# 959AI994/Multi-Gate-VAE

Hardware: NVIDIA B200
Metric: gates_per_s_fwd_bwd (higher is better)
Workload: dtype f32

## Files before the change

multi-gate-vae_b200/csrc/linear.cu:

```cuda
#include "mgv_common.cuh"

namespace {

constexpr int RG = 8;

template <int TO, int TI, int LR>
__global__ void __launch_bounds__(256) linear_wgrad_kernel(const float* __restrict__ x, const float* __restrict__ gy, long long N,
                                                           int I, int O, int IP, int OP, float* __restrict__ partial) {
    extern __shared__ __align__(16) float sm[];
    const int stage_floats = LR * (IP + OP);
    const int tid = threadIdx.x, nt = blockDim.x;
    const int ntx = IP / TI, tx = tid % ntx, ty = tid / ntx;
    const bool active = ty < OP / TO;
    float acc[TO][TI];
    float bsum[TO];
#pragma unroll
    for (int a = 0; a < TO; ++a) {
        bsum[a] = 0.f;
#pragma unroll
        for (int b = 0; b < TI; ++b) acc[a][b] = 0.f;
    }
    const long long trips = (N + LR - 1) / LR;
    const long long t0 = trips * blockIdx.x / gridDim.x, t1 = trips * (blockIdx.x + 1) / gridDim.x;
    const bool vec = (I == IP) && (O == OP) && (I % 4 == 0) && (O % 4 == 0);
    auto stage = [&](long long t, int buf) {
        float* Xs = sm + buf * stage_floats;
        float* Gs = Xs + LR * IP;
        const long long r0 = t * LR;
        const int rows = (int)((N - r0 < LR) ? (N - r0) : LR);
        if (vec) {
            const float* xs = x + r0 * I;
            const float* gs = gy + r0 * O;
            for (int q = tid; q < LR * I / 4; q += nt) {
                const unsigned src = (q < rows * I / 4) ? 16u : 0u;
                asm volatile("cp.async.cg.shared.global [%0], [%1], 16, %2;" ::"r"((unsigned)__cvta_generic_to_shared(Xs + 4 * q)),
                             "l"(src ? xs + 4 * q : x), "r"(src) : "memory");
            }
            for (int q = tid; q < LR * O / 4; q += nt) {
                const unsigned src = (q < rows * O / 4) ? 16u : 0u;
                asm volatile("cp.async.cg.shared.global [%0], [%1], 16, %2;" ::"r"((unsigned)__cvta_generic_to_shared(Gs + 4 * q)),
                             "l"(src ? gs + 4 * q : gy), "r"(src) : "memory");
            }
        } else {
            for (int q = tid; q < LR * IP; q += nt) {
                const int r = q / IP, c = q % IP;
                Xs[q] = (r < rows && c < I) ? x[(r0 + r) * I + c] : 0.f;
            }
            for (int q = tid; q < LR * OP; q += nt) {
                const int r = q / OP, c = q % OP;
                Gs[q] = (r < rows && c < O) ? gy[(r0 + r) * O + c] : 0.f;
            }
        }
        asm volatile("cp.async.commit_group;" ::: "memory");
    };
    if (t0 < t1) stage(t0, 0);
    for (long long t = t0; t < t1; ++t) {
        const int buf = (int)((t - t0) & 1);
        if (t + 1 < t1) {
            stage(t + 1, buf ^ 1);
            asm volatile("cp.async.wait_group 1;" ::: "memory");
        } else {
            asm volatile("cp.async.wait_group 0;" ::: "memory");
        }
        __syncthreads();
        const float* Xs = sm + buf * stage_floats;
        const float* Gs = Xs + LR * IP;
        if (active) {
#pragma unroll 4
            for (int r = 0; r < LR; ++r) {
                float g[TO], xv[TI];
#pragma unroll
                for (int a = 0; a < TO; a += 4) *reinterpret_cast<float4*>(&g[a]) = *reinterpret_cast<const float4*>(Gs + r * OP + TO * ty + a);
#pragma unroll
                for (int b = 0; b < TI; b += 4) *reinterpret_cast<float4*>(&xv[b]) = *reinterpret_cast<const float4*>(Xs + r * IP + (b / 4) * (IP / 2) + 4 * tx);
#pragma unroll
                for (int a = 0; a < TO; ++a) {
                    bsum[a] += g[a];
#pragma unroll
                    for (int b = 0; b < TI; ++b) acc[a][b] = fmaf(g[a], xv[b], acc[a][b]);
                }
            }
        }
        __syncthreads();
    }
    if (!active) return;
    float* P = partial + (size_t)blockIdx.x * ((size_t)O * I + O);
#pragma unroll
    for (int a = 0; a < TO; ++a) {
        const int o = TO * ty + a;
        if (o < O) {
#pragma unroll
            for (int b = 0; b < TI; ++b) {
                const int i = (b / 4) * (IP / 2) + 4 * tx + (b & 3);
                if (i < I) P[(size_t)o * I + i] = acc[a][b];
            }
            if (tx == 0) P[(size_t)O * I + o] = bsum[a];
        }
    }
}

__global__ void __launch_bounds__(256) linear_wgrad_reduce_kernel(const float* __restrict__ partial, int nblk, int I, int O,
                                                                  float* __restrict__ dW, float* __restrict__ db) {
    __shared__ float red[RG][32];
    const int total = O * I + O;
    const int j = threadIdx.x & 31, g = threadIdx.x >> 5;
    const int i = blockIdx.x * 32 + j;
    float s = 0.f;
    if (i < total) {
#pragma unroll 4
        for (int b = g; b < nblk; b += RG) s += partial[(size_t)b * total + i];
    }
    red[g][j] = s;
    __syncthreads();
    if (g == 0 && i < total) {
#pragma unroll
        for (int k = 1; k < RG; ++k) s += red[k][j];
        if (i < O * I) dW[i] = s;
        else if (db) db[i - O * I] = s;
    }
}

int grid_blocks(long long N) {
    int dev = 0, sms = 148;
    cudaGetDevice(&dev);
    cudaDeviceGetAttribute(&sms, cudaDevAttrMultiProcessorCount, dev);
    long long trips = (N + 127) / 128;
    long long g = 2LL * sms;
    if (g > trips) g = trips;
    return g < 1 ? 1 : (int)g;
}

template <int TO, int TI, int LR>
int launch(int nblk, cudaStream_t st, const float* x, const float* gy, long long N, int I, int O, float* partial) {
    const int IP = (I + TI - 1) / TI * TI, OP = (O + TO - 1) / TO * TO;
    int nt = (IP / TI) * (OP / TO);
    nt = nt < 256 ? 256 : (nt + 31) / 32 * 32;
    const size_t smem = 2 * (size_t)LR * (IP + OP) * sizeof(float);
    MGV_CUDA(cudaFuncSetAttribute((const void*)linear_wgrad_kernel<TO, TI, LR>, cudaFuncAttributeMaxDynamicSharedMemorySize, (int)smem));
    linear_wgrad_kernel<TO, TI, LR><<<nblk, nt, smem, st>>>(x, gy, N, I, O, IP, OP, partial);
    return MGV_OK;
}

}

extern "C" size_t mgv_linear_wgrad_workspace_bytes(int64_t N, int32_t I, int32_t O) {
    return (size_t)grid_blocks(N) * ((size_t)O * I + O) * sizeof(float) + 256;
}

extern "C" int mgv_linear_wgrad(const float* x, const float* gy, int64_t N, int32_t I, int32_t O, float* dW, float* db,
                                void* ws, size_t ws_bytes, mgv_stream_t stream) {
    cudaStream_t st = (cudaStream_t)stream;
    MGV_REQUIRE(I >= 1 && I <= 128 && O >= 1 && O <= 128, "mgv_linear_wgrad: in/out features must be in 1..128 (got %d, %d)", I, O);
    MGV_REQUIRE(N >= 0 && dW != nullptr, "mgv_linear_wgrad: bad argument");
    if (N == 0) {
        MGV_CUDA(cudaMemsetAsync(dW, 0, (size_t)O * I * sizeof(float), st));
        if (db) MGV_CUDA(cudaMemsetAsync(db, 0, (size_t)O * sizeof(float), st));
        return MGV_OK;
    }
    if (ws_bytes < mgv_linear_wgrad_workspace_bytes(N, I, O)) {
        mgv_set_error("mgv_linear_wgrad: workspace %zu < %zu bytes", ws_bytes, mgv_linear_wgrad_workspace_bytes(N, I, O));
        return MGV_ERR_WORKSPACE;
    }
    const int nblk = grid_blocks(N);
    float* partial = (float*)ws;
    const bool o8 = O > 32, i8 = I > 32;
    int rc;
    if (o8 && i8) rc = launch<8, 8, 64>(nblk, st, x, gy, N, I, O, partial);
    else if (o8) rc = launch<8, 4, 128>(nblk, st, x, gy, N, I, O, partial);
    else if (i8) rc = launch<4, 8, 128>(nblk, st, x, gy, N, I, O, partial);
    else rc = launch<4, 4, 128>(nblk, st, x, gy, N, I, O, partial);
    if (rc != MGV_OK) return rc;
    const int total = O * I + O;
    linear_wgrad_reduce_kernel<<<(total + 31) / 32, 256, 0, st>>>(partial, nblk, I, O, dW, db);
    mgv_count_launches(2);
    return mgv_check_cuda(cudaGetLastError(), "mgv_linear_wgrad");
}
```

multi-gate-vae_b200/csrc/readout.cu:

```cuda
#include "mgv_common.cuh"

namespace {

constexpr int DI = MGV_D, DH = 32;
constexpr int RD_THREADS = 256, RD_WARPS = RD_THREADS / 32;
constexpr int NB = 4;

struct RdParams {
    const float *W1, *b1, *g1, *be1, *W2, *b2, *g2, *be2, *W3, *b3;
    float *rm1, *rv1, *rm2, *rv2;
};
struct RdFwd {
    RdParams P;
    const float* x; long long N;
    int training; float p_drop; unsigned long long seed; float momentum, eps;
    const float* target;
    float* pred; float* loss;
    float* saved;
    float* stats;
    unsigned* mask;
    double* acc;
    unsigned* bar;
};
struct RdBwd {
    RdParams P;
    const float* x; long long N;
    int training; float p_drop; unsigned long long seed;
    const float* target; const float* saved; const float* stats;
    const float* g_pred;
    const float* g_loss;
    float* gx;
    float* grads;
    float* dz1;
    float* partial;
    double* acc;
    unsigned* bar;
};
constexpr int G_W1 = 0, G_B1 = 2048, G_G1 = 2080, G_BE1 = 2112, G_W2 = 2144, G_B2 = 3168, G_G2 = 3200, G_BE2 = 3232, G_W3 = 3264, G_B3 = 3296;

__device__ __forceinline__ float keep_scale(unsigned long long seed, long long n, int layer, int c, float p, float sc) {
    if (p <= 0.f) return 1.0f;
    uint32_t h = (uint32_t)(n * 64 + layer * 32 + c) ^ (uint32_t)seed;
    h ^= h >> 16; h *= 0x85EBCA6Bu; h ^= h >> 13; h *= 0xC2B2AE35u; h ^= h >> 16;
    h += (uint32_t)(seed >> 32) + (uint32_t)(n >> 26);
    h ^= h >> 15; h *= 0x2C1B3C6Du; h ^= h >> 12; h *= 0x297A2D39u; h ^= h >> 15;
    const float u = (float)(h >> 8) * (1.0f / 16777216.0f);
    return u >= p ? sc : 0.f;
}
__device__ __forceinline__ float warp_sum(float v) {
#pragma unroll
    for (int o = 16; o > 0; o >>= 1) v += __shfl_xor_sync(0xffffffffu, v, o);
    return v;
}
__device__ __forceinline__ float dot64(const float* xs, const float (&w)[DI], float b) {
    float a0 = b, a1 = 0.f;
#pragma unroll
    for (int k = 0; k < DI; k += 4) {
        const float4 v = *reinterpret_cast<const float4*>(xs + k);
        a0 = fmaf(v.x, w[k], a0); a1 = fmaf(v.y, w[k + 1], a1);
        a0 = fmaf(v.z, w[k + 2], a0); a1 = fmaf(v.w, w[k + 3], a1);
    }
    return a0 + a1;
}
__device__ __forceinline__ float dot32(float h, const float (&w)[DH], float b) {
    float a0 = b, a1 = 0.f;
#pragma unroll
    for (int j = 0; j < DH; j += 2) {
        a0 = fmaf(__shfl_sync(0xffffffffu, h, j), w[j], a0);
        a1 = fmaf(__shfl_sync(0xffffffffu, h, j + 1), w[j + 1], a1);
    }
    return a0 + a1;
}

__global__ void __launch_bounds__(RD_THREADS, 2) readout_fwd_kernel(const RdFwd p) {
    __shared__ __align__(16) float xs[RD_WARPS][NB][DI];
    __shared__ double red[RD_WARPS][2][DH];
    const int lane = threadIdx.x & 31, warp = threadIdx.x >> 5;
    const long long gw = (long long)blockIdx.x * RD_WARPS + warp, nw = (long long)gridDim.x * RD_WARPS;
    const RdParams& P = p.P;
    const float sc = p.p_drop > 0.f ? 1.0f / (1.0f - p.p_drop) : 1.0f;
    const bool train = p.training != 0;
    float w[DI];
#pragma unroll
    for (int k = 0; k < DI; ++k) w[k] = __ldg(P.W1 + lane * DI + k);
    const float b1 = __ldg(P.b1 + lane);
    double s = 0.0, q = 0.0;
    for (long long n0 = gw * NB; n0 < p.N; n0 += nw * NB) {
#pragma unroll
        for (int i = 0; i < NB; ++i)
            if (n0 + i < p.N) *reinterpret_cast<float2*>(&xs[warp][i][2 * lane]) = __ldg(reinterpret_cast<const float2*>(p.x + (n0 + i) * DI) + lane);
        __syncwarp();
#pragma unroll
        for (int i = 0; i < NB; ++i) {
            if (n0 + i < p.N) {
                const float y = dot64(xs[warp][i], w, b1);
                p.saved[(n0 + i) * 64 + lane] = y;
                s += (double)y; q += (double)y * (double)y;
            }
        }
        __syncwarp();
    }
    float mean1, is1;
    if (train) {
        red[warp][0][lane] = s; red[warp][1][lane] = q;
        __syncthreads();
        if (warp == 0) {
            double a = 0.0, b = 0.0;
            for (int v = 0; v < RD_WARPS; ++v) { a += red[v][0][lane]; b += red[v][1][lane]; }
            atomicAdd(p.acc + lane, a); atomicAdd(p.acc + DH + lane, b);
        }
        mgv_grid_sync(p.bar, gridDim.x);
        const double m = __ldcg(p.acc + lane) / (double)p.N;
        const double var = fmax(__ldcg(p.acc + DH + lane) / (double)p.N - m * m, 0.0);
        mean1 = (float)m; is1 = (float)(1.0 / sqrt(var + (double)p.eps));
        if (blockIdx.x == 0 && warp == 0) {
            p.stats[lane] = mean1; p.stats[DH + lane] = is1;
            const double unb = p.N > 1 ? var * (double)p.N / (double)(p.N - 1) : var;
            P.rm1[lane] = (1.0f - p.momentum) * P.rm1[lane] + p.momentum * mean1;
            P.rv1[lane] = (1.0f - p.momentum) * P.rv1[lane] + p.momentum * (float)unb;
        }
    } else {
        mean1 = __ldg(P.rm1 + lane); is1 = rsqrtf(__ldg(P.rv1 + lane) + p.eps);
        if (blockIdx.x == 0 && warp == 0) { p.stats[lane] = mean1; p.stats[DH + lane] = is1; }
    }
    float w2[DH];
#pragma unroll
    for (int j = 0; j < DH; ++j) w2[j] = __ldg(P.W2 + lane * DH + j);
    const float g1 = __ldg(P.g1 + lane) * is1, o1 = __ldg(P.be1 + lane) - mean1 * g1, b2 = __ldg(P.b2 + lane);
    s = 0.0; q = 0.0;
    for (long long n0 = gw * NB; n0 < p.N; n0 += nw * NB) {
        float y1[NB], k1[NB], y2[NB];
#pragma unroll
        for (int i = 0; i < NB; ++i) y1[i] = (n0 + i < p.N) ? p.saved[(n0 + i) * 64 + lane] : 0.f;
#pragma unroll
        for (int i = 0; i < NB; ++i) k1[i] = train ? keep_scale(p.seed, n0 + i, 0, lane, p.p_drop, sc) : 1.0f;
#pragma unroll
        for (int i = 0; i < NB; ++i) y2[i] = dot32(fmaxf(fmaf(y1[i], g1, o1), 0.f) * k1[i], w2, b2);
#pragma unroll
        for (int i = 0; i < NB; ++i) {
            if (n0 + i < p.N) {
                p.saved[(n0 + i) * 64 + DH + lane] = y2[i];
                s += (double)y2[i]; q += (double)y2[i] * (double)y2[i];
            }
            if (p.mask) {
                const unsigned bits = __ballot_sync(0xffffffffu, k1[i] != 0.f);
                if (lane == 0 && n0 + i < p.N) p.mask[(n0 + i) * 2] = bits;
            }
        }
    }
    float mean2, is2;
    if (train) {
        __syncthreads();
        red[warp][0][lane] = s; red[warp][1][lane] = q;
        __syncthreads();
        if (warp == 0) {
            double a = 0.0, b = 0.0;
            for (int v = 0; v < RD_WARPS; ++v) { a += red[v][0][lane]; b += red[v][1][lane]; }
            atomicAdd(p.acc + 2 * DH + lane, a); atomicAdd(p.acc + 3 * DH + lane, b);
        }
        mgv_grid_sync(p.bar, gridDim.x);
        const double m = __ldcg(p.acc + 2 * DH + lane) / (double)p.N;
        const double var = fmax(__ldcg(p.acc + 3 * DH + lane) / (double)p.N - m * m, 0.0);
        mean2 = (float)m; is2 = (float)(1.0 / sqrt(var + (double)p.eps));
        if (blockIdx.x == 0 && warp == 0) {
            p.stats[2 * DH + lane] = mean2; p.stats[3 * DH + lane] = is2;
            const double unb = p.N > 1 ? var * (double)p.N / (double)(p.N - 1) : var;
            P.rm2[lane] = (1.0f - p.momentum) * P.rm2[lane] + p.momentum * mean2;
            P.rv2[lane] = (1.0f - p.momentum) * P.rv2[lane] + p.momentum * (float)unb;
        }
    } else {
        mean2 = __ldg(P.rm2 + lane); is2 = rsqrtf(__ldg(P.rv2 + lane) + p.eps);
        if (blockIdx.x == 0 && warp == 0) { p.stats[2 * DH + lane] = mean2; p.stats[3 * DH + lane] = is2; }
    }
    const float g2 = __ldg(P.g2 + lane) * is2, o2 = __ldg(P.be2 + lane) - mean2 * g2, w3 = __ldg(P.W3 + lane), b3 = __ldg(P.b3);
    double lsum = 0.0;
    for (long long n0 = gw * NB; n0 < p.N; n0 += nw * NB) {
        float y2[NB], k2[NB], y3[NB];
#pragma unroll
        for (int i = 0; i < NB; ++i) y2[i] = (n0 + i < p.N) ? p.saved[(n0 + i) * 64 + DH + lane] : 0.f;
#pragma unroll
        for (int i = 0; i < NB; ++i) k2[i] = train ? keep_scale(p.seed, n0 + i, 1, lane, p.p_drop, sc) : 1.0f;
#pragma unroll
        for (int i = 0; i < NB; ++i) y3[i] = fmaxf(fmaf(y2[i], g2, o2), 0.f) * k2[i] * w3;
#pragma unroll
        for (int o = 16; o > 0; o >>= 1)
#pragma unroll
            for (int i = 0; i < NB; ++i) y3[i] += __shfl_xor_sync(0xffffffffu, y3[i], o);
#pragma unroll
        for (int i = 0; i < NB; ++i) {
            const long long n = n0 + i;
            const float pr = fminf(fmaxf(y3[i] + b3, 0.f), 1.f);
            if (p.mask) {
                const unsigned bits = __ballot_sync(0xffffffffu, k2[i] != 0.f);
                if (lane == 0 && n < p.N) p.mask[n * 2 + 1] = bits;
            }
            if (lane == 0 && n < p.N) {
                p.pred[n] = pr;
                if (p.target) lsum += (double)fabsf(pr - __ldg(p.target + n));
            }
        }
    }
    if (p.target) {
        __syncthreads();
        if (lane == 0) red[warp][0][0] = lsum;
        __syncthreads();
        if (threadIdx.x == 0) {
            double a = 0.0;
            for (int v = 0; v < RD_WARPS; ++v) a += red[v][0][0];
            atomicAdd(p.acc + 4 * DH, a);
        }
        mgv_grid_sync(p.bar, gridDim.x);
        if (blockIdx.x == 0 && threadIdx.x == 0) p.loss[0] = (float)(__ldcg(p.acc + 4 * DH) / (double)(p.N > 0 ? p.N : 1));
    }
}

template <int NV>
__device__ __forceinline__ void block_tree_add(float (&v)[NV], float* scratch, int warp, int lane) {
#pragma unroll 1
    for (int half = RD_WARPS / 2; half >= 1; half >>= 1) {
        if (warp >= half && warp < 2 * half) {
#pragma unroll
            for (int i = 0; i < NV; ++i) scratch[((warp - half) * NV + i) * 32 + lane] = v[i];
        }
        __syncthreads();
        if (warp < half) {
#pragma unroll
            for (int i = 0; i < NV; ++i) v[i] += scratch[(warp * NV + i) * 32 + lane];
        }
        __syncthreads();
    }
}
constexpr int RD_SCRATCH_BYTES = (RD_WARPS / 2) * 65 * 32 * 4;

__global__ void __launch_bounds__(RD_THREADS, 2) readout_bwd_kernel(const RdBwd p) {
    __shared__ __align__(16) float xs[RD_WARPS][NB][DI];
    __shared__ __align__(16) float W1s[DH][DI];
    __shared__ double red[RD_WARPS][2][DH];
    extern __shared__ __align__(16) float scratch[];
    const int lane = threadIdx.x & 31, warp = threadIdx.x >> 5;
    const long long gw = (long long)blockIdx.x * RD_WARPS + warp, nw = (long long)gridDim.x * RD_WARPS;
    const RdParams& P = p.P;
    const bool train = p.training != 0;
    const float sc = (train && p.p_drop > 0.f) ? 1.0f / (1.0f - p.p_drop) : 1.0f;
    const float pd = train ? p.p_drop : 0.f;
    float* part = p.partial + (size_t)blockIdx.x * 3297;
    for (int i = threadIdx.x; i < DH * DI; i += RD_THREADS) W1s[i / DI][i % DI] = __ldg(P.W1 + i);
    __syncthreads();
    const float mean1 = p.stats[lane], is1 = p.stats[DH + lane], mean2 = p.stats[2 * DH + lane], is2 = p.stats[3 * DH + lane];
    const float g1 = __ldg(P.g1 + lane), be1 = __ldg(P.be1 + lane), g2 = __ldg(P.g2 + lane), be2 = __ldg(P.be2 + lane);
    const float w3 = __ldg(P.W3 + lane), b3 = __ldg(P.b3);
    const float gl = p.g_loss ? __ldg(p.g_loss) / (float)(p.N > 0 ? p.N : 1) : 0.f;
    const double invN = 1.0 / (double)(p.N > 0 ? p.N : 1);

    auto dz2_group = [&](long long n0, float (&xh2)[NB], float (&h2)[NB], float (&dp)[NB], float (&dz2)[NB]) {
        float y2[NB], k2[NB], d[NB], tg[NB], a2[NB], y3[NB];
#pragma unroll
        for (int i = 0; i < NB; ++i) {
            const long long n = n0 + i;
            const bool ok = n < p.N;
            y2[i] = ok ? p.saved[n * 64 + DH + lane] : 0.f;
            d[i] = (ok && p.g_pred) ? __ldg(p.g_pred + n) : 0.f;
            tg[i] = (ok && p.target) ? __ldg(p.target + n) : 0.f;
        }
#pragma unroll
        for (int i = 0; i < NB; ++i) k2[i] = keep_scale(p.seed, n0 + i, 1, lane, pd, sc);
#pragma unroll
        for (int i = 0; i < NB; ++i) {
            xh2[i] = (y2[i] - mean2) * is2;
            a2[i] = fmaf(xh2[i], g2, be2);
            h2[i] = fmaxf(a2[i], 0.f) * k2[i];
            y3[i] = h2[i] * w3;
        }
#pragma unroll
        for (int o = 16; o > 0; o >>= 1)
#pragma unroll
            for (int i = 0; i < NB; ++i) y3[i] += __shfl_xor_sync(0xffffffffu, y3[i], o);
#pragma unroll
        for (int i = 0; i < NB; ++i) {
            const float y = y3[i] + b3;
            const float pr = fminf(fmaxf(y, 0.f), 1.f);
            float dd = d[i];
            if (p.target) {
                const float diff = pr - tg[i];
                dd += gl * (diff > 0.f ? 1.f : (diff < 0.f ? -1.f : 0.f));
            }
            dp[i] = (n0 + i < p.N && y >= 0.f && y <= 1.f) ? dd : 0.f;
            dz2[i] = a2[i] > 0.f ? dp[i] * w3 * k2[i] : 0.f;
        }
    };
    {
        double sa = 0.0, sb = 0.0;
        float dw3 = 0.f, db3 = 0.f;
        for (long long n0 = gw * NB; n0 < p.N; n0 += nw * NB) {
            float xh2[NB], h2[NB], dp[NB], dz2[NB];
            dz2_group(n0, xh2, h2, dp, dz2);
#pragma unroll
            for (int i = 0; i < NB; ++i) {
                dw3 = fmaf(dp[i], h2[i], dw3); db3 += dp[i];
                sa += (double)dz2[i]; sb += (double)dz2[i] * (double)xh2[i];
            }
        }
        {
            float v[4] = {dw3, db3, (float)sa, (float)sb};
            block_tree_add<4>(v, scratch, warp, lane);
            if (warp == 0) {
                part[G_W3 + lane] = v[0];
                if (lane == 0) part[G_B3] = v[1];
                part[G_BE2 + lane] = v[2]; part[G_G2 + lane] = v[3];
            }
        }
        red[warp][0][lane] = sa; red[warp][1][lane] = sb;
        __syncthreads();
        if (warp == 0) {
            double a = 0.0, b = 0.0;
            for (int v = 0; v < RD_WARPS; ++v) { a += red[v][0][lane]; b += red[v][1][lane]; }
            atomicAdd(p.acc + lane, a); atomicAdd(p.acc + DH + lane, b);
        }
        mgv_grid_sync(p.bar, gridDim.x);
    }
    {
        const float s2a = train ? (float)(__ldcg(p.acc + lane) * invN) : 0.f, s2b = train ? (float)(__ldcg(p.acc + DH + lane) * invN) : 0.f;
        float w2t[DH], dw2[DH];
#pragma unroll
        for (int c = 0; c < DH; ++c) { w2t[c] = __ldg(P.W2 + c * DH + lane); dw2[c] = 0.f; }
        float db2 = 0.f;
        double sa = 0.0, sb = 0.0;
        for (long long n0 = gw * NB; n0 < p.N; n0 += nw * NB) {
            float xh2[NB], h2[NB], dp[NB], dz2[NB];
            float y1[NB];
#pragma unroll
            for (int i = 0; i < NB; ++i) y1[i] = (n0 + i < p.N) ? p.saved[(n0 + i) * 64 + lane] : 0.f;
            dz2_group(n0, xh2, h2, dp, dz2);
            float dy2[NB], xh1[NB], a1[NB], k1[NB], h1[NB], dh1[NB];
#pragma unroll
            for (int i = 0; i < NB; ++i) {
                dy2[i] = (n0 + i < p.N) ? g2 * is2 * (dz2[i] - s2a - xh2[i] * s2b) : 0.f;
                db2 += dy2[i];
                xh1[i] = (y1[i] - mean1) * is1;
                a1[i] = fmaf(xh1[i], g1, be1);
                k1[i] = keep_scale(p.seed, n0 + i, 0, lane, pd, sc);
                h1[i] = fmaxf(a1[i], 0.f) * k1[i];
                dh1[i] = 0.f;
            }
#pragma unroll
            for (int c = 0; c < DH; ++c) {
#pragma unroll
                for (int i = 0; i < NB; ++i) {
                    const float dyc = __shfl_sync(0xffffffffu, dy2[i], c);
                    dh1[i] = fmaf(dyc, w2t[c], dh1[i]);
                    dw2[c] = fmaf(dyc, h1[i], dw2[c]);
                }
            }
#pragma unroll
            for (int i = 0; i < NB; ++i) {
                if (n0 + i < p.N) {
                    const float dz1 = a1[i] > 0.f ? dh1[i] * k1[i] : 0.f;
                    p.dz1[(n0 + i) * DH + lane] = dz1;
                    sa += (double)dz1; sb += (double)dz1 * (double)xh1[i];
                }
            }
        }
        {
            float v[DH + 3];
#pragma unroll
            for (int c = 0; c < DH; ++c) v[c] = dw2[c];
            v[DH] = db2; v[DH + 1] = (float)sa; v[DH + 2] = (float)sb;
            block_tree_add<DH + 3>(v, scratch, warp, lane);
            if (warp == 0) {
#pragma unroll
                for (int c = 0; c < DH; ++c) part[G_W2 + c * DH + lane] = v[c];
                part[G_B2 + lane] = v[DH]; part[G_BE1 + lane] = v[DH + 1]; part[G_G1 + lane] = v[DH + 2];
            }
        }
        red[warp][0][lane] = sa; red[warp][1][lane] = sb;
        __syncthreads();
        if (warp == 0) {
            double a = 0.0, b = 0.0;
            for (int v = 0; v < RD_WARPS; ++v) { a += red[v][0][lane]; b += red[v][1][lane]; }
            atomicAdd(p.acc + 2 * DH + lane, a); atomicAdd(p.acc + 3 * DH + lane, b);
        }
        mgv_grid_sync(p.bar, gridDim.x);
    }
    {
        const float s1a = train ? (float)(__ldcg(p.acc + 2 * DH + lane) * invN) : 0.f, s1b = train ? (float)(__ldcg(p.acc + 3 * DH + lane) * invN) : 0.f;
        float dw1[DI];
#pragma unroll
        for (int k = 0; k < DI; ++k) dw1[k] = 0.f;
        float db1 = 0.f;
        for (long long n0 = gw * NB; n0 < p.N; n0 += nw * NB) {
#pragma unroll
            for (int i = 0; i < NB; ++i)
                if (n0 + i < p.N) *reinterpret_cast<float2*>(&xs[warp][i][2 * lane]) = __ldg(reinterpret_cast<const float2*>(p.x + (n0 + i) * DI) + lane);
            __syncwarp();
#pragma unroll 1
            for (int i = 0; i < NB; ++i) {
                const long long n = n0 + i;
                if (n >= p.N) break;
                const float xh1 = (p.saved[n * 64 + lane] - mean1) * is1;
                const float dy1 = g1 * is1 * (p.dz1[n * DH + lane] - s1a - xh1 * s1b);
                db1 += dy1;
#pragma unroll
                for (int k = 0; k < DI; k += 4) {
                    const float4 v = *reinterpret_cast<const float4*>(&xs[warp][i][k]);
                    dw1[k] = fmaf(dy1, v.x, dw1[k]); dw1[k + 1] = fmaf(dy1, v.y, dw1[k + 1]);
                    dw1[k + 2] = fmaf(dy1, v.z, dw1[k + 2]); dw1[k + 3] = fmaf(dy1, v.w, dw1[k + 3]);
                }
                float2 dx = make_float2(0.f, 0.f);
#pragma unroll
                for (int c = 0; c < DH; ++c) {
                    const float dyc = __shfl_sync(0xffffffffu, dy1, c);
                    const float2 wv = *reinterpret_cast<const float2*>(&W1s[c][2 * lane]);
                    dx.x = fmaf(dyc, wv.x, dx.x); dx.y = fmaf(dyc, wv.y, dx.y);
                }
                *reinterpret_cast<float2*>(p.gx + n * DI + 2 * lane) = dx;
            }
            __syncwarp();
        }
        {
            float v[DI + 1];
#pragma unroll
            for (int k = 0; k < DI; ++k) v[k] = dw1[k];
            v[DI] = db1;
            block_tree_add<DI + 1>(v, scratch, warp, lane);
            if (warp == 0) {
#pragma unroll
                for (int k = 0; k < DI; ++k) part[G_W1 + lane * DI + k] = v[k];
                part[G_B1 + lane] = v[DI];
            }
        }
    }
    mgv_grid_sync(p.bar, gridDim.x);
    for (int i = blockIdx.x * RD_THREADS + threadIdx.x; i < 3297; i += gridDim.x * RD_THREADS) {
        float t = 0.f;
        for (unsigned b = 0; b < gridDim.x; ++b) t += __ldcg(p.partial + (size_t)b * 3297 + i);
        p.grads[i] = t;
    }
}

int fill_params(RdParams& P, const void* const* params) {
    MGV_REQUIRE(params != nullptr, "readout: null parameter table");
    for (int i = 0; i < 14; ++i) MGV_REQUIRE(params[i] != nullptr, "readout: parameter %d is null", i);
    P.W1 = (const float*)params[0]; P.b1 = (const float*)params[1]; P.g1 = (const float*)params[2]; P.be1 = (const float*)params[3];
    P.rm1 = (float*)params[4]; P.rv1 = (float*)params[5];
    P.W2 = (const float*)params[6]; P.b2 = (const float*)params[7]; P.g2 = (const float*)params[8]; P.be2 = (const float*)params[9];
    P.rm2 = (float*)params[10]; P.rv2 = (float*)params[11];
    P.W3 = (const float*)params[12]; P.b3 = (const float*)params[13];
    return MGV_OK;
}

int coop_blocks(const void* kern, long long N, int* out, size_t dyn_smem = 0) {
    int dev = 0, sms = 0, occ = 0;
    MGV_CUDA(cudaGetDevice(&dev));
    MGV_CUDA(cudaDeviceGetAttribute(&sms, cudaDevAttrMultiProcessorCount, dev));
    if (dyn_smem) MGV_CUDA(cudaFuncSetAttribute(kern, cudaFuncAttributeMaxDynamicSharedMemorySize, (int)dyn_smem));
    MGV_CUDA(cudaOccupancyMaxActiveBlocksPerMultiprocessor(&occ, kern, RD_THREADS, dyn_smem));
    MGV_REQUIRE(occ >= 1, "readout: kernel does not fit on an SM");
    long long want = (N + RD_WARPS * NB - 1) / (RD_WARPS * NB);
    const long long cap = (long long)sms * (occ > 2 ? 2 : occ);
    *out = (int)(want < 1 ? 1 : (want > cap ? cap : want));
    return MGV_OK;
}

}

constexpr int RD_MAX_BLOCKS = 1024;
extern "C" size_t mgv_readout_workspace_bytes(int64_t N) {
    return mgv_align_up((size_t)(N > 0 ? N : 1) * DH * 4 + 256, 256) + mgv_align_up(192 * sizeof(double), 256) +
           mgv_align_up((size_t)RD_MAX_BLOCKS * 3297 * 4 + 256, 256) + 1024;
}

extern "C" int mgv_readout_fwd(const float* x, int64_t N, const void* const* params, int32_t training, float p_drop, uint64_t seed,
                               float momentum, float eps, const float* target, float* pred, float* loss, float* saved, float* stats,
                               uint32_t* mask, void* ws, size_t ws_bytes, int32_t* sync, mgv_stream_t stream) {
    cudaStream_t st = (cudaStream_t)stream;
    MGV_REQUIRE(N >= 0 && pred && saved && stats && sync && (N == 0 || x), "mgv_readout_fwd: bad argument");
    MGV_REQUIRE(!target || loss, "mgv_readout_fwd: a target needs the loss output");
    MGV_REQUIRE(p_drop >= 0.f && p_drop < 1.f, "mgv_readout_fwd: p_drop must be in [0, 1)");
    if (ws_bytes < mgv_readout_workspace_bytes(N)) { mgv_set_error("mgv_readout_fwd: workspace too small"); return MGV_ERR_WORKSPACE; }
    RdFwd p{};
    int rc = fill_params(p.P, params);
    if (rc != MGV_OK) return rc;
    MgvArena a(ws, ws_bytes);
    (void)a.take<float>((size_t)(N > 0 ? N : 1) * DH);
    p.acc = a.take<double>(192);
    p.x = x; p.N = N; p.training = training; p.p_drop = training ? p_drop : 0.f; p.seed = seed; p.momentum = momentum; p.eps = eps;
    p.target = target; p.pred = pred; p.loss = loss; p.saved = saved; p.stats = stats; p.mask = mask;
    p.bar = reinterpret_cast<unsigned*>(sync);
    MGV_CUDA(cudaMemsetAsync(p.acc, 0, 192 * sizeof(double), st));
    MGV_CUDA(cudaMemsetAsync(sync, 0, sizeof(int32_t), st));
    if (N == 0) {
        if (loss) MGV_CUDA(cudaMemsetAsync(loss, 0, sizeof(float), st));
        return MGV_OK;
    }
    int blocks = 0;
    rc = coop_blocks((const void*)readout_fwd_kernel, N, &blocks);
    if (rc != MGV_OK) return rc;
    void* args[] = {&p};
    MGV_CUDA(cudaLaunchCooperativeKernel((const void*)readout_fwd_kernel, dim3(blocks), dim3(RD_THREADS), args, 0, st));
    mgv_count_launches(1);
    return MGV_OK;
}

extern "C" int mgv_readout_bwd(const float* x, int64_t N, const void* const* params, int32_t training, float p_drop, uint64_t seed,
                               const float* target, const float* saved, const float* stats, const float* g_pred, const float* g_loss,
                               float* gx, float* grads, void* ws, size_t ws_bytes, int32_t* sync, mgv_stream_t stream) {
    cudaStream_t st = (cudaStream_t)stream;
    MGV_REQUIRE(N >= 0 && saved && stats && gx && grads && sync && (N == 0 || x), "mgv_readout_bwd: bad argument");
    MGV_REQUIRE(!g_loss || target, "mgv_readout_bwd: a loss gradient needs the target");
    if (ws_bytes < mgv_readout_workspace_bytes(N)) { mgv_set_error("mgv_readout_bwd: workspace too small"); return MGV_ERR_WORKSPACE; }
    RdBwd p{};
    int rc = fill_params(p.P, params);
    if (rc != MGV_OK) return rc;
    MgvArena a(ws, ws_bytes);
    p.dz1 = a.take<float>((size_t)(N > 0 ? N : 1) * DH);
    p.acc = a.take<double>(192);
    p.partial = a.take<float>((size_t)RD_MAX_BLOCKS * 3297);
    p.x = x; p.N = N; p.training = training; p.p_drop = p_drop; p.seed = seed;
    p.target = g_loss ? target : nullptr; p.saved = saved; p.stats = stats; p.g_pred = g_pred; p.g_loss = g_loss;
    p.gx = gx; p.grads = grads; p.bar = reinterpret_cast<unsigned*>(sync);
    MGV_CUDA(cudaMemsetAsync(p.acc, 0, 192 * sizeof(double), st));
    MGV_CUDA(cudaMemsetAsync(sync, 0, sizeof(int32_t), st));
    if (N == 0) {
        MGV_CUDA(cudaMemsetAsync(grads, 0, 3297 * sizeof(float), st));
        return MGV_OK;
    }
    int blocks = 0;
    rc = coop_blocks((const void*)readout_bwd_kernel, N, &blocks, (size_t)RD_SCRATCH_BYTES);
    if (rc != MGV_OK) return rc;
    MGV_REQUIRE(blocks <= RD_MAX_BLOCKS, "mgv_readout_bwd: grid of %d blocks exceeds the partial buffer", blocks);
    void* args[] = {&p};
    MGV_CUDA(cudaLaunchCooperativeKernel((const void*)readout_bwd_kernel, dim3(blocks), dim3(RD_THREADS), args, (size_t)RD_SCRATCH_BYTES, st));
    mgv_count_launches(1);
    return MGV_OK;
}
```

Baseline: 18.97 million.

## Use split-fp16 tensor-core MMA for linear weight gradient; prefetch readout rows to smem

Adds a tensor-core weight-gradient kernel for 64/128-wide layers. It splits fp32 inputs into hi/lo 16-bit pairs with per-tile power-of-two rescaling to approximate fp32 accuracy, and it becomes the default unless an env var selects the old FFMA path. The aim is to replace scalar FMA work with MMA throughput, at the cost of extra split and scale work and a per-tile block sync. Separately, the readout backward now stages the saved activations and dz1 rows into shared memory together with x, so the global loads are issued as a batch before the dependent per-row loop.

```diff
diff --git a/multi-gate-vae_b200/csrc/linear.cu b/multi-gate-vae_b200/csrc/linear.cu
--- a/multi-gate-vae_b200/csrc/linear.cu
+++ b/multi-gate-vae_b200/csrc/linear.cu
@@ -1,4 +1,7 @@
+#include <stdlib.h>
+#include <string.h>
 #include "mgv_common.cuh"
+#include "mgv_mma16.cuh"
 
 namespace {
 
@@ -141,6 +144,136 @@
     return MGV_OK;
 }
 
+constexpr int MK_ROWS = 64;
+
+template <int O, int I>
+struct MmaShape {
+    static constexpr int WM = O / 32, WN = I / 32, THREADS = 32 * WM * WN;
+    static constexpr int LDG = O + 8, LDX = I + 8;
+    static constexpr int GV = MK_ROWS * O / 4 / THREADS, XV = MK_ROWS * I / 4 / THREADS;
+    static constexpr int G_HI = 0, G_LO = G_HI + MK_ROWS * LDG * 2, X_HI = G_LO + MK_ROWS * LDG * 2, X_LO = X_HI + MK_ROWS * LDX * 2;
+    static constexpr int RED = X_LO + MK_ROWS * LDX * 2;
+    static constexpr int SMEM = RED + 2 * WM * WN * 4;
+    static_assert(GV >= 1 && XV >= 1 && THREADS % (O / 4) == 0 && THREADS % (I / 4) == 0, "tile split");
+    static_assert(THREADS * 4 * 4 <= SMEM, "bias reduction reuses the planes");
+};
+
+template <int O, int I>
+__global__ void __launch_bounds__(MmaShape<O, I>::THREADS, 512 / MmaShape<O, I>::THREADS) linear_wgrad_mma_kernel(const float* __restrict__ x, const float* __restrict__ gy,
+                                                                                   long long N, float* __restrict__ partial) {
+    using S = MmaShape<O, I>;
+    extern __shared__ __align__(128) unsigned char smem[];
+    const uint32_t sb = m16::smem_u32(smem);
+    float* red = reinterpret_cast<float*>(smem + S::RED);
+    const int tid = threadIdx.x, lane = tid & 31, warp = tid >> 5;
+    const int wm = warp / S::WN, wn = warp % S::WN;
+    const int gc = tid % (O / 4), gr = tid / (O / 4), xc = tid % (I / 4), xr = tid / (I / 4);
+    constexpr int GSTEP = S::THREADS / (O / 4), XSTEP = S::THREADS / (I / 4);
+    const long long tiles = (N + MK_ROWS - 1) / MK_ROWS;
+    const long long t0 = tiles * blockIdx.x / gridDim.x, t1 = tiles * (blockIdx.x + 1) / gridDim.x;
+    float4 gv[S::GV], xv[S::XV];
+    auto load = [&](long long t) {
+        const long long r0 = t * MK_ROWS;
+#pragma unroll
+        for (int j = 0; j < S::GV; ++j) {
+            const long long r = r0 + gr + j * GSTEP;
+            gv[j] = r < N ? __ldg(reinterpret_cast<const float4*>(gy + r * O) + gc) : make_float4(0.f, 0.f, 0.f, 0.f);
+        }
+#pragma unroll
+        for (int j = 0; j < S::XV; ++j) {
+            const long long r = r0 + xr + j * XSTEP;
+            xv[j] = r < N ? __ldg(reinterpret_cast<const float4*>(x + r * I) + xc) : make_float4(0.f, 0.f, 0.f, 0.f);
+        }
+    };
+    float c[2][4][4];
+    m16::zero_frag(c);
+    float bsum[4] = {0.f, 0.f, 0.f, 0.f};
+    float sg = 1.0f, sx = 1.0f;
+    const int n0[4] = {32 * wn, 32 * wn + 8, 32 * wn + 16, 32 * wn + 24};
+    if (t0 < t1) load(t0);
+    for (long long t = t0; t < t1; ++t) {
+        float ag = 0.f, ax = 0.f;
+#pragma unroll
+        for (int j = 0; j < S::GV; ++j) ag = fmaxf(ag, fmaxf(fmaxf(fabsf(gv[j].x), fabsf(gv[j].y)), fmaxf(fabsf(gv[j].z), fabsf(gv[j].w))));
+#pragma unroll
+        for (int j = 0; j < S::XV; ++j) ax = fmaxf(ax, fmaxf(fmaxf(fabsf(xv[j].x), fabsf(xv[j].y)), fmaxf(fabsf(xv[j].z), fabsf(xv[j].w))));
+#pragma unroll
+        for (int o = 16; o > 0; o >>= 1) {
+            ag = fmaxf(ag, __shfl_xor_sync(0xffffffffu, ag, o));
+            ax = fmaxf(ax, __shfl_xor_sync(0xffffffffu, ax, o));
+        }
+        if (lane == 0) { red[warp] = ag; red[S::WM * S::WN + warp] = ax; }
+        __syncthreads();
+        ag = 0.f; ax = 0.f;
+#pragma unroll
+        for (int w = 0; w < S::WM * S::WN; ++w) { ag = fmaxf(ag, red[w]); ax = fmaxf(ax, red[S::WM * S::WN + w]); }
+        const float ng = m16::pow2_scale_keep(ag, sg), nx = m16::pow2_scale_keep(ax, sx);
+        if (ng != sg) { m16::scale_frag(c, ng / sg); sg = ng; }
+        if (nx != sx) { m16::scale_frag(c, nx / sx); sx = nx; }
+#pragma unroll
+        for (int j = 0; j < S::GV; ++j) {
+            bsum[0] += gv[j].x; bsum[1] += gv[j].y; bsum[2] += gv[j].z; bsum[3] += gv[j].w;
+            uint2 hi, lo;
+            m16::split2(gv[j].x * sg, gv[j].y * sg, hi.x, lo.x);
+            m16::split2(gv[j].z * sg, gv[j].w * sg, hi.y, lo.y);
+            const int off = ((gr + j * GSTEP) * S::LDG + 4 * gc) * 2;
+            *reinterpret_cast<uint2*>(smem + S::G_HI + off) = hi;
+            *reinterpret_cast<uint2*>(smem + S::G_LO + off) = lo;
+        }
+#pragma unroll
+        for (int j = 0; j < S::XV; ++j) {
+            uint2 hi, lo;
+            m16::split2(xv[j].x * sx, xv[j].y * sx, hi.x, lo.x);
+            m16::split2(xv[j].z * sx, xv[j].w * sx, hi.y, lo.y);
+            const int off = ((xr + j * XSTEP) * S::LDX + 4 * xc) * 2;
+            *reinterpret_cast<uint2*>(smem + S::X_HI + off) = hi;
+            *reinterpret_cast<uint2*>(smem + S::X_LO + off) = lo;
+        }
+        if (t + 1 < t1) load(t + 1);
+        __syncthreads();
+        m16::warp_gemm<2, 4, MK_ROWS / 16, true, true>(c, sb + S::G_HI, sb + S::G_LO, S::LDG, 32 * wm, 0, sb + S::X_HI, sb + S::X_LO,
+                                                       S::LDX, n0, 0, lane);
+    }
+    float* P = partial + (size_t)blockIdx.x * ((size_t)O * I + O);
+    const float inv = (1.0f / sg) * (1.0f / sx);
+    const int g = lane >> 2, q = lane & 3;
+#pragma unroll
+    for (int mt = 0; mt < 2; ++mt)
+#pragma unroll
+        for (int nt = 0; nt < 4; ++nt)
+#pragma unroll
+            for (int h = 0; h < 2; ++h) {
+                const int o = 32 * wm + 16 * mt + g + 8 * h, i = n0[nt] + 2 * q;
+                *reinterpret_cast<float2*>(P + (size_t)o * I + i) = make_float2(c[mt][nt][2 * h] * inv, c[mt][nt][2 * h + 1] * inv);
+            }
+    __syncthreads();
+    float4* bs = reinterpret_cast<float4*>(smem);
+    bs[tid] = make_float4(bsum[0], bsum[1], bsum[2], bsum[3]);
+    __syncthreads();
+    if (tid < O / 4) {
+        float4 a = bs[tid];
+        for (int k = 1; k < GSTEP; ++k) {
+            const float4 b = bs[tid + k * (O / 4)];
+            a.x += b.x; a.y += b.y; a.z += b.z; a.w += b.w;
+        }
+        *reinterpret_cast<float4*>(P + (size_t)O * I + 4 * tid) = a;
+    }
+}
+
+template <int O, int I>
+int launch_mma(int nblk, cudaStream_t st, const float* x, const float* gy, long long N, float* partial) {
+    using S = MmaShape<O, I>;
+    MGV_CUDA(cudaFuncSetAttribute((const void*)linear_wgrad_mma_kernel<O, I>, cudaFuncAttributeMaxDynamicSharedMemorySize, S::SMEM));
+    linear_wgrad_mma_kernel<O, I><<<nblk, S::THREADS, S::SMEM, st>>>(x, gy, N, partial);
+    return MGV_OK;
+}
+
+bool use_mma(int I, int O, const float* x, const float* gy) {
+    const char* e = getenv("MGV_LINEAR_WGRAD");
+    if (e && !strcmp(e, "ffma")) return false;
+    return (I == 64 || I == 128) && (O == 64 || O == 128) && ((uintptr_t)x % 16 == 0) && ((uintptr_t)gy % 16 == 0);
+}
+
 }
 
 extern "C" size_t mgv_linear_wgrad_workspace_bytes(int64_t N, int32_t I, int32_t O) {
@@ -165,7 +298,10 @@
     float* partial = (float*)ws;
     const bool o8 = O > 32, i8 = I > 32;
     int rc;
-    if (o8 && i8) rc = launch<8, 8, 64>(nblk, st, x, gy, N, I, O, partial);
+    if (use_mma(I, O, x, gy)) {
+        if (O == 64) rc = I == 64 ? launch_mma<64, 64>(nblk, st, x, gy, N, partial) : launch_mma<64, 128>(nblk, st, x, gy, N, partial);
+        else rc = I == 64 ? launch_mma<128, 64>(nblk, st, x, gy, N, partial) : launch_mma<128, 128>(nblk, st, x, gy, N, partial);
+    } else if (o8 && i8) rc = launch<8, 8, 64>(nblk, st, x, gy, N, I, O, partial);
     else if (o8) rc = launch<8, 4, 128>(nblk, st, x, gy, N, I, O, partial);
     else if (i8) rc = launch<4, 8, 128>(nblk, st, x, gy, N, I, O, partial);
     else rc = launch<4, 4, 128>(nblk, st, x, gy, N, I, O, partial);
diff --git a/multi-gate-vae_b200/csrc/readout.cu b/multi-gate-vae_b200/csrc/readout.cu
--- a/multi-gate-vae_b200/csrc/readout.cu
+++ b/multi-gate-vae_b200/csrc/readout.cu
@@ -235,6 +235,7 @@
 __global__ void __launch_bounds__(RD_THREADS, 2) readout_bwd_kernel(const RdBwd p) {
     __shared__ __align__(16) float xs[RD_WARPS][NB][DI];
     __shared__ __align__(16) float W1s[DH][DI];
+    __shared__ float y1s[RD_WARPS][NB][DH], dzs[RD_WARPS][NB][DH];
     __shared__ double red[RD_WARPS][2][DH];
     extern __shared__ __align__(16) float scratch[];
     const int lane = threadIdx.x & 31, warp = threadIdx.x >> 5;
@@ -389,15 +390,20 @@
         float db1 = 0.f;
         for (long long n0 = gw * NB; n0 < p.N; n0 += nw * NB) {
 #pragma unroll
-            for (int i = 0; i < NB; ++i)
-                if (n0 + i < p.N) *reinterpret_cast<float2*>(&xs[warp][i][2 * lane]) = __ldg(reinterpret_cast<const float2*>(p.x + (n0 + i) * DI) + lane);
+            for (int i = 0; i < NB; ++i) {
+                if (n0 + i < p.N) {
+                    *reinterpret_cast<float2*>(&xs[warp][i][2 * lane]) = __ldg(reinterpret_cast<const float2*>(p.x + (n0 + i) * DI) + lane);
+                    y1s[warp][i][lane] = p.saved[(n0 + i) * 64 + lane];
+                    dzs[warp][i][lane] = p.dz1[(n0 + i) * DH + lane];
+                }
+            }
             __syncwarp();
 #pragma unroll 1
             for (int i = 0; i < NB; ++i) {
                 const long long n = n0 + i;
                 if (n >= p.N) break;
-                const float xh1 = (p.saved[n * 64 + lane] - mean1) * is1;
-                const float dy1 = g1 * is1 * (p.dz1[n * DH + lane] - s1a - xh1 * s1b);
+                const float xh1 = (y1s[warp][i][lane] - mean1) * is1;
+                const float dy1 = g1 * is1 * (dzs[warp][i][lane] - s1a - xh1 * s1b);
                 db1 += dy1;
 #pragma unroll
                 for (int k = 0; k < DI; k += 4) {
```

Measured after the change: 19.21 million (median of 6 runs). Within noise of the previous version (+1.2%).
